# kjenike/panagram

Measured on AMD Instinct MI355X. Metric: anchored k-mers/sec building pan-kmer bitmap, higher is better.
Workload: dtype u64

## Files before the change

panagram_amd/csrc/pg_api.hip:

```cpp
#include "pg_host.h"

thread_local std::string pg::g_err;

int pg::fail(int code, const char *fmt, ...) {
    char buf[512];
    va_list ap;
    va_start(ap, fmt);
    vsnprintf(buf, sizeof buf, fmt, ap);
    va_end(ap);
    g_err = buf;
    return code;
}

extern "C" const char *pg_last_error(void) { return g_err.c_str(); }
int pg_set_error(int code, const char *msg) {
    g_err = msg ? msg : "";
    return code;
}
extern "C" const char *pg_version(void) { return "panagram_hip 0.2 gfx950"; }
extern "C" uint32_t pg_tile_positions(void) { return (uint32_t)PROBE_TILE; }

int pg::use_device(const pg_ctx *c) {
    HIP_TRY(hipSetDevice(c->device));
    return PG_OK;
// ... 699 lines not shown
    }
    return fail(PG_E_CAPACITY, "k-mer counting table keeps overflowing");
    PG_API_END
}

static int insert_keys_dev(pg_table *t, int db_idx, const uint64_t *d_keys, const uint32_t *d_vals, uint64_t n) {
    const int si = 0, w = db_idx;
    if (int r = ensure_room(t, si, n)) return r;
    for (int attempt = 0; attempt < 8; ++attempt) {
        hipStream_t st = t->ctx->stream;
        HIP_TRY(hipMemsetAsync(t->d_counters, 0, 2 * sizeof(unsigned long long), st));
        HIP_TRY(launch_insert_keys(st, t->subs[si].d, w, d_keys, d_vals, n, t->d_counters, MAX_PROBE));
        unsigned long long cnt[2];
        if (int r = read_counters(t, cnt)) return r;
        t->subs[si].count += cnt[0];
        if (cnt[1] == 0) return after_insert(t, si);
        if (int r = grow_after_overflow(t, si, n)) return r;
    }
    return fail(PG_E_CAPACITY, "k-mer table keeps overflowing");
}

extern "C" int pg_table_insert_keys(pg_table *t, int db_idx, const uint64_t *keys, const uint32_t *counters,
                                    uint64_t n) {
    PG_API_BEGIN
    if (!t || (n && (!keys || !counters))) return fail(PG_E_INVALID, "pg_table_insert_keys: NULL argument");
    if (db_idx < 0 || db_idx >= t->ndbs) return fail(PG_E_INVALID, "db index %d out of range (0..%d)", db_idx, t->ndbs - 1);
    if (n == 0) return PG_OK;
    if (int r = use_device(t->ctx)) return r;
    TABLE_WRITER(t);
    DevBuf<uint64_t> dk;
    DevBuf<uint32_t> dv;
    hipError_t e = dk.alloc(n);
    if (e == hipSuccess) e = dv.alloc(n);
    if (e != hipSuccess) return fail(PG_E_HIP, "hipMalloc failed: %s", hipGetErrorString(e));
    int r = PG_OK;
    if (hipMemcpyAsync(dk.get(), keys, n * 8, hipMemcpyHostToDevice, t->ctx->stream) != hipSuccess ||
        hipMemcpyAsync(dv.get(), counters, n * 4, hipMemcpyHostToDevice, t->ctx->stream) != hipSuccess)
        r = fail(PG_E_HIP, "H2D copy of keys failed");
    if (!r) r = insert_keys_dev(t, db_idx, dk.get(), dv.get(), n);
    hipStreamSynchronize(t->ctx->stream);
    return r;
    PG_API_END
}

extern "C" int pg_table_stats(pg_table *t, uint64_t *nkeys, uint64_t *nslots, uint64_t *nbuckets, uint64_t *bytes) {
    PG_API_BEGIN
    if (!t) return fail(PG_E_INVALID, "table is NULL");
    uint64_t a = 0, b = 0, c = 0;
    for (auto &s : t->subs) {
        a += s.count;
        b += s.d.nbuckets * s.d.slots;
        c += s.d.nbuckets;
    }
    if (nkeys) *nkeys = a;
    if (nslots) *nslots = b;
    if (nbuckets) *nbuckets = c;
    if (bytes) {
        uint64_t by = 0;
        for (auto &s2 : t->subs) by += table_bytes(s2.d);
        *bytes = by;
    }
    return PG_OK;
    PG_API_END
}

static int count_spill(pg_table *t, int si, uint64_t *out) {
    hipStream_t st = t->ctx->stream;
    HIP_TRY(hipMemsetAsync(t->d_counters, 0, 2 * sizeof(unsigned long long), st));
    HIP_TRY(launch_count_spill(st, t->subs[si].d, t->d_counters));
    unsigned long long c[2];
    if (int r = read_counters(t, c)) return r;
    *out = c[0];
    return PG_OK;
}

extern "C" int pg_table_rehash(pg_table *t, double keys_per_bucket) {
    PG_API_BEGIN
    if (!t) return fail(PG_E_INVALID, "table is NULL");
    if (!(keys_per_bucket > 0.05 && keys_per_bucket <= 8.0)) return fail(PG_E_INVALID, "keys_per_bucket must be in (0.05, 8]");
    if (int r = use_device(t->ctx)) return r;
    TABLE_WRITER(t);
    if (!t->m_pinned) {
        uint64_t most = 0;
        for (auto &s : t->subs) most = std::max<uint64_t>(most, s.count);
        t->m = minimizer_length((uint32_t)t->k, most, t->max_len, window_cap(t->ngenomes), (uint32_t)t->ngenomes, t->cosched);
    }
    uint32_t slots = 8;
    if (const char *e = getenv("PG_TABLE_SLOTS"))
        if (atoi(e) == 16) slots = 16;
    uint64_t keys = 0, spilled = 0;
    for (size_t si = 0; si < t->subs.size(); ++si) {
        if (t->subs[si].d.layout != LAYOUT_SLOTS) slots = t->subs[si].d.slots;
        const double kpb = std::min(keys_per_bucket * (slots / 8.0), 0.8 * slots);
        if (int r = regrow(t, (int)si, (uint64_t)((double)t->subs[si].count / kpb) + 1, slots)) return r;
        uint64_t sp = 0;
        if (int r = count_spill(t, (int)si, &sp)) return r;
        keys += t->subs[si].count;
        spilled += sp;
    }
    t->spill = keys ? (double)spilled / (double)keys : 0.0;
    return PG_OK;
    PG_API_END
}

extern "C" int pg_table_measure_spill(pg_table *t, double *fraction) {
    PG_API_BEGIN
    if (!t) return fail(PG_E_INVALID, "table is NULL");
    if (int r = use_device(t->ctx)) return r;
    TABLE_WRITER(t);
    uint64_t keys = 0, spilled = 0;
    for (size_t si = 0; si < t->subs.size(); ++si) {
        uint64_t sp = 0;
        if (int r = count_spill(t, (int)si, &sp)) return r;
        keys += t->subs[si].count;
        spilled += sp;
    }
    if (fraction) *fraction = keys ? (double)spilled / (double)keys : 0.0;
    return PG_OK;
    PG_API_END
}

extern "C" int pg_table_spill(const pg_table *t, double *fraction, uint32_t *slots) {
    PG_API_BEGIN
    if (!t) return fail(PG_E_INVALID, "table is NULL");
    if (fraction) *fraction = t->spill;
    if (slots) *slots = t->subs.empty() ? 0 : t->subs[0].d.slots;
    return PG_OK;
    PG_API_END
}

extern "C" int pg_table_export(pg_table *t, int db_idx, uint64_t *keys, uint32_t *counters, uint64_t cap, uint64_t *n) {
    PG_API_BEGIN
    if (!t || !n) return fail(PG_E_INVALID, "pg_table_export: NULL argument");
    if (db_idx < 0 || db_idx >= t->ndbs) return fail(PG_E_INVALID, "db index %d out of range", db_idx);
    if (int r = use_device(t->ctx)) return r;
    const int si = 0, w = db_idx;
    hipStream_t st = t->ctx->stream;
    DevBuf<uint64_t> dk;
    DevBuf<uint32_t> dv;
    if (keys && cap) {
        hipError_t e = dk.alloc(cap);
        if (e == hipSuccess) e = dv.alloc(cap);
        if (e != hipSuccess) return fail(PG_E_HIP, "hipMalloc failed: %s", hipGetErrorString(e));
    }
    int rc = PG_OK;
    unsigned long long cnt[2] = {0, 0};
    if (hipMemsetAsync(t->d_counters, 0, 16, st) != hipSuccess ||
        launch_export(st, t->subs[si].d, w, dk.get(), dv.get(), dk.get() ? cap : 0, t->d_counters) != hipSuccess)
        rc = fail(PG_E_HIP, "export kernel failed");
    if (!rc) rc = read_counters(t, cnt);
    if (!rc && dk.get()) {
        uint64_t m = std::min<uint64_t>(cnt[0], cap);
        if (hipMemcpy(keys, dk.get(), m * 8, hipMemcpyDeviceToHost) != hipSuccess ||
            hipMemcpy(counters, dv.get(), m * 4, hipMemcpyDeviceToHost) != hipSuccess)
            rc = fail(PG_E_HIP, "D2H copy failed");
    }
    *n = cnt[0];
    return rc;
    PG_API_END
}

static TableDesc make_desc(const pg_table *t) {
    TableDesc T;
    memset(&T, 0, sizeof T);
    T.nsub = (uint32_t)t->subs.size();
    for (uint32_t i = 0; i < T.nsub; ++i) T.sub[i] = t->subs[i].d;
    T.ndbs = t->ndbs;
    T.k = t->k;
    T.ngenomes = t->ngenomes;
    return T;
}

struct ResultGeom {
    uint32_t lowres_step = 100;
    uint64_t max_bin_len = 200000;
    uint32_t min_bin_count = 100;
};

static int result_create(pg_ctx *ctx, pg_table *t, int k, uint32_t N, const pg_seqset *sq, uint32_t flags,
                         const ResultGeom &geo, pg_result **out) {
    if (ctx != sq->ctx) return fail(PG_E_INVALID, "table / context and seqset belong to different contexts");
    if (geo.lowres_step < 1 || geo.max_bin_len < 1 || geo.min_bin_count < 1)
        return fail(PG_E_INVALID, "lowres_step, max_bin_len and min_bin_count must be >= 1");
    if (int r = use_device(ctx)) return r;
    const uint32_t nbytes = (N + 7) / 8;
    pg_result *r = new pg_result();
    r->ctx = ctx;
    r->tbl = t;
    r->seqs = sq;
    r->N = N;
    r->k = k;
    if (t) ++t->refs;
    else ++ctx->refs;
    ++const_cast<pg_seqset *>(sq)->refs;
    r->flags = flags;
    r->lowres_step = geo.lowres_step;
    r->d_ad = nullptr;
    r->d_tile_contig = nullptr;
    r->d_out1 = r->d_out100 = nullptr;
    r->d_bins = nullptr;
    r->d_colsums = nullptr;
    r->ev_ok = r->ev_epi = false;
    for (auto &e : r->ev) e = nullptr;
    uint64_t o1 = 0, o100 = 0, bins = 0, tiles = 0;
    std::vector<uint32_t> tile_contig;
    for (uint32_t c = 0; c < sq->n; ++c) {
        const uint64_t len = sq->desc[c].len;
        const uint64_t nk = len >= (uint64_t)k ? len - k + 1 : 0;
        if (nk > 0xFFFFFFF0ull) {
            pg_result_destroy(r);
            return fail(PG_E_INVALID, "contig %u has %llu k-mers; contigs must stay below 2^32 (as in KMC)", c, (unsigned long long)nk);
        }
        AnchorDesc a;
        a.nkmers = (uint32_t)nk;
        uint64_t binlen = geo.max_bin_len;
        if (nk / binlen < geo.min_bin_count) binlen = nk / geo.min_bin_count;
        if (binlen == 0) binlen = 1;
        a.binlen = (uint32_t)binlen;
        a.nbins = (uint32_t)((nk + binlen - 1) / binlen);
        a.out_off = o1;
        a.out100_off = o100;
        a.bin_off = bins;
        a.tile0 = (uint32_t)tiles;
        const uint64_t n100 = (nk + geo.lowres_step - 1) / geo.lowres_step;
        r->nrows100.push_back(n100);
        o1 += (nk * nbytes + 15) & ~15ull;
        o100 += n100 * nbytes;
        bins += a.nbins;
        const uint64_t nt = (nk + PROBE_TILE - 1) / PROBE_TILE;
        for (uint64_t i = 0; i < nt; ++i) tile_contig.push_back(c);
        tiles += nt;
        r->ad.push_back(a);
    }
    if (tiles > 0x7FFFFFFFull) {
        pg_result_destroy(r);
        return fail(PG_E_INVALID, "too many tiles in one launch");
    }
    r->ntiles = (uint32_t)tiles;
    r->out1_bytes = o1;
    r->out100_bytes = o100;
    r->total_bins = bins;
    hipStream_t st = ctx->stream;
    hipError_t e;
    if ((e = hipMalloc(reinterpret_cast<void **>(&r->d_ad), std::max<size_t>(1, r->ad.size()) * sizeof(AnchorDesc))) == hipSuccess &&
        (e = hipMalloc(reinterpret_cast<void **>(&r->d_tile_contig), std::max<size_t>(1, tile_contig.size()) * 4)) == hipSuccess &&
        (e = row_alloc(ctx, (flags & PG_ANCHOR_COLUMNS_ONLY) ? 16 : std::max<uint64_t>(16, o1) + 16, &r->d_out1, &r->out1_cap)) == hipSuccess &&
        (e = hipMalloc(reinterpret_cast<void **>(&r->d_out100), std::max<uint64_t>(16, o100))) == hipSuccess &&
        (e = hipMalloc(reinterpret_cast<void **>(&r->d_bins), std::max<uint64_t>(1, bins) * (N + 1) * 4)) == hipSuccess &&
        (e = hipMalloc(reinterpret_cast<void **>(&r->d_colsums), std::max<size_t>(1, r->ad.size()) * N * 8)) == hipSuccess) {
        if (!r->ad.empty())
            e = hipMemcpyAsync(r->d_ad, r->ad.data(), r->ad.size() * sizeof(AnchorDesc), hipMemcpyHostToDevice, st);
        if (e == hipSuccess && !tile_contig.empty())
            e = hipMemcpyAsync(r->d_tile_contig, tile_contig.data(), tile_contig.size() * 4, hipMemcpyHostToDevice, st);
        if (e == hipSuccess && !t) e = hipMemsetAsync(r->d_out1, 0, std::max<uint64_t>(16, o1), st);
        if (e == hipSuccess) e = hipStreamSynchronize(st);
    }
    if (e != hipSuccess) {
        pg_result_destroy(r);
        return fail(PG_E_HIP, "result allocation failed: %s", hipGetErrorString(e));
    }
    *out = r;
    return PG_OK;
}

extern "C" int pg_result_create(pg_table *t, const pg_seqset *sq, uint32_t flags, pg_result **out) {
    PG_API_BEGIN
    if (!t || !sq || !out) return fail(PG_E_INVALID, "pg_result_create: NULL argument");
    return result_create(t->ctx, t, t->k, (uint32_t)t->ngenomes, sq, flags, ResultGeom(), out);
    PG_API_END
}

extern "C" int pg_result_create_ex(pg_table *t, const pg_seqset *sq, uint32_t flags, uint32_t lowres_step,
                                   uint64_t max_bin_len, uint32_t min_bin_count, pg_result **out) {
    PG_API_BEGIN
    if (!t || !sq || !out) return fail(PG_E_INVALID, "pg_result_create_ex: NULL argument");
    ResultGeom g;
    g.lowres_step = lowres_step;
    g.max_bin_len = max_bin_len;
    g.min_bin_count = min_bin_count;
    return result_create(t->ctx, t, t->k, (uint32_t)t->ngenomes, sq, flags, g, out);
    PG_API_END
}

extern "C" int pg_result_create_rows(pg_ctx *ctx, int k, int ngenomes, const pg_seqset *sq, uint32_t flags,
                                     uint32_t lowres_step, uint64_t max_bin_len, uint32_t min_bin_count, pg_result **out) {
    PG_API_BEGIN
    if (!ctx || !sq || !out) return fail(PG_E_INVALID, "pg_result_create_rows: NULL argument");
    if (k < 1 || k > 32) return fail(PG_E_INVALID, "k=%d unsupported (1..32)", k);
    if (ngenomes < 1) return fail(PG_E_INVALID, "ngenomes must be >= 1");
    ResultGeom g;
    g.lowres_step = lowres_step;
    g.max_bin_len = max_bin_len;
    g.min_bin_count = min_bin_count;
    return result_create(ctx, nullptr, k, (uint32_t)ngenomes, sq, flags | PG_ANCHOR_ROWS_ONLY, g, out);
    PG_API_END
}

extern "C" int pg_result_destroy(pg_result *r) {
    PG_API_BEGIN
    if (!r) return PG_OK;
    hipSetDevice(r->ctx->device);
    hipStreamSynchronize(r->ctx->stream);
    hipStreamSynchronize(r->ctx->aux_stream);
    hipFree(r->d_ad);
    hipFree(r->d_tile_contig);
    row_free(r->ctx, r->d_out1, r->out1_cap);
    hipFree(r->d_out100);
    hipFree(r->d_bins);
    hipFree(r->d_colsums);
    if (r->d_sched) hipFree(r->d_sched);
    if (r->d_ranges) hipFree(r->d_ranges);
    if (r->d_tile_hist) hipFree(r->d_tile_hist);
    if (r->d_tile_cs) hipFree(r->d_tile_cs);
    if (r->d_small) hipFree(r->d_small);
    for (auto e : r->chunk_ev) hipEventDestroy(e);
    for (auto *v : {&r->ev_hist, &r->ev_free})
        for (auto &s : *v)
            for (auto &e : s.e)
                if (e) hipEventDestroy(e);
    pg_table *t = r->tbl;
    pg_ctx *c = r->ctx;
    pg_seqset *sq = const_cast<pg_seqset *>(r->seqs);
    delete r;
    if (t) table_release(t);
    else ctx_release(c);
    seqset_release(sq);
    return PG_OK;
    PG_API_END
}

static int build_chunks(pg_result *r, const uint32_t *sched) {
    r->chunks.clear();
    r->chunks_ready = true;
    if (r->d_ranges) {
        hipFree(r->d_ranges);
        r->d_ranges = nullptr;
    }
    const char *env = getenv("PG_RUN_CHUNKS");
    const uint32_t nbytes = (r->N + 7) / 8;
    uint32_t K = env ? (uint32_t)atoi(env) : ((nbytes == 8 && r->ntiles >= (4u << 20)) ? 16u : 1u);
    const char *mt = getenv("PG_CHUNK_MIN_TILES");
    K = std::min(K, r->ntiles / std::max(1u, mt ? (uint32_t)atoi(mt) : 32768u));
    if (K < 2) return PG_OK;
    std::vector<uint2> ranges;
    for (uint32_t c = 0; c < K; ++c) {
        pg_result::Chunk ch;
        ch.s0 = (uint32_t)((uint64_t)r->ntiles * c / K);
        ch.s1 = (uint32_t)((uint64_t)r->ntiles * (c + 1) / K);
        ch.r0 = (uint32_t)ranges.size();
        ch.tiles = ch.s1 - ch.s0;
        if (!sched) {
            ranges.push_back(make_uint2(ch.s0, ch.s1));
        } else {
            std::vector<uint2> runs;
            for (uint32_t i = ch.s0; i < ch.s1; ++i) {
                if (!runs.empty() && runs.back().y == sched[i]) ++runs.back().y;
                else runs.push_back(make_uint2(sched[i], sched[i] + 1));
            }
            std::sort(runs.begin(), runs.end(), [](const uint2 &a, const uint2 &b) { return a.x < b.x; });
            for (const uint2 &u : runs) {
                if (ranges.size() > ch.r0 && ranges.back().y == u.x) ranges.back().y = u.y;
                else ranges.push_back(u);
            }
        }
        ch.nr = (uint32_t)ranges.size() - ch.r0;
        if (ch.nr > 512) {
            r->chunks.clear();
            return PG_OK;
        }
        r->chunks.push_back(ch);
    }
    HIP_TRY(hipMalloc(reinterpret_cast<void **>(&r->d_ranges), ranges.size() * sizeof(uint2)));
    HIP_TRY(hipMemcpy(r->d_ranges, ranges.data(), ranges.size() * sizeof(uint2), hipMemcpyHostToDevice));
    while (r->chunk_ev.size() < r->chunks.size()) {
        hipEvent_t e;
        HIP_TRY(hipEventCreateWithFlags(&e, hipEventDisableTiming));
        r->chunk_ev.push_back(e);
    }
    return PG_OK;
}

static int coschedule(pg_result *r, const uint32_t *contig_group, uint32_t piece_tiles, const uint32_t *range_first,
                      uint32_t nranges, const uint32_t *contig_class = nullptr) {
    if (int e = use_device(r->ctx)) return e;
    hipStream_t st = r->ctx->stream;
    HIP_TRY(hipStreamSynchronize(st));
    HIP_TRY(hipStreamSynchronize(r->ctx->aux_stream));
    if (r->d_sched) {
        hipFree(r->d_sched);
        r->d_sched = nullptr;
    }
    r->sched_bounds.clear();
    r->chunks.clear();
    r->chunks_ready = false;
    if (!contig_group || r->ntiles == 0) return PG_OK;
    const bool auto_piece = piece_tiles == 0;
    const size_t nc = r->ad.size();
    std::vector<uint32_t> firsts;
    if (range_first && nranges) {
        for (uint32_t i = 0; i < nranges; ++i) {
            if (range_first[i] >= nc || (i && range_first[i] <= range_first[i - 1]) || (!i && range_first[0] != 0))
                return fail(PG_E_INVALID, "pg_result_coschedule_ranges: range starts must begin at contig 0 and increase");
            firsts.push_back(range_first[i]);
        }
    } else {
        firsts.push_back(0);
    }
    firsts.push_back((uint32_t)nc);
    struct Piece {
        double at;
        uint32_t g, first;
    };
    std::vector<uint32_t> sched;
    sched.reserve(r->ntiles);
    std::vector<std::vector<uint32_t>> members;
    if (contig_class) {
        std::vector<std::pair<uint32_t, uint32_t>> byclass;
        for (size_t c = 0; c < nc; ++c) byclass.emplace_back(contig_class[c], (uint32_t)c);
        std::stable_sort(byclass.begin(), byclass.end(), [](auto &x, auto &y) { return x.first < y.first; });
        for (size_t i = 0; i < byclass.size(); ++i) {
            if (i == 0 || byclass[i].first != byclass[i - 1].first) members.emplace_back();
            members.back().push_back(byclass[i].second);
        }
        r->sched_bounds.push_back(0);
    } else {
        for (size_t ri = 0; ri + 1 < firsts.size(); ++ri) {
            members.emplace_back();
            for (uint32_t c = firsts[ri]; c < firsts[ri + 1]; ++c) members.back().push_back(c);
            r->sched_bounds.push_back(r->ad[firsts[ri]].tile0);
        }
    }
    for (const auto &mem : members) {
        uint32_t ngroups = 0;
        for (uint32_t c : mem) ngroups = std::max(ngroups, contig_group[c] + 1);
        std::vector<std::vector<uint32_t>> tiles(ngroups);
        for (uint32_t c : mem) {
            const uint32_t nt = (uint32_t)(((uint64_t)r->ad[c].nkmers + PROBE_TILE - 1) / PROBE_TILE);
            for (uint32_t i = 0; i < nt; ++i) tiles[contig_group[c]].push_back(r->ad[c].tile0 + i);
        }
        if (auto_piece) piece_tiles = ngroups <= 32 ? 64u : std::max(8u, 512u / ngroups);
        std::vector<Piece> pieces;
        for (uint32_t g = 0; g < ngroups; ++g) {
            const size_t np = (tiles[g].size() + piece_tiles - 1) / piece_tiles;
            for (size_t i = 0; i < np; ++i) pieces.push_back({(double)i / (double)np, g, (uint32_t)(i * piece_tiles)});
        }
        std::stable_sort(pieces.begin(), pieces.end(), [](const Piece &x, const Piece &y) { return x.at < y.at; });
        for (const Piece &p : pieces) {
            const size_t end = std::min<size_t>(tiles[p.g].size(), (size_t)p.first + piece_tiles);
            for (size_t i = p.first; i < end; ++i) sched.push_back(tiles[p.g][i]);
        }
    }
    r->sched_bounds.push_back(r->ntiles);
    if (sched.size() != r->ntiles) return fail(PG_E_INVALID, "internal: schedule does not cover the tiles");
    HIP_TRY(hipMalloc(reinterpret_cast<void **>(&r->d_sched), (size_t)r->ntiles * 4));
    HIP_TRY(hipMemcpyAsync(r->d_sched, sched.data(), (size_t)r->ntiles * 4, hipMemcpyHostToDevice, st));
    HIP_TRY(hipStreamSynchronize(st));
    if (!(r->flags & PG_ANCHOR_ROWS_ONLY)) return build_chunks(r, sched.data());
    return PG_OK;
}

extern "C" int pg_result_coschedule(pg_result *r, const uint32_t *contig_group, uint32_t piece_tiles) {
    PG_API_BEGIN
    if (!r) return fail(PG_E_INVALID, "result is NULL");
    return coschedule(r, contig_group, piece_tiles, nullptr, 0);
    PG_API_END
}

extern "C" int pg_result_coschedule_classes(pg_result *r, const uint32_t *contig_group, const uint32_t *contig_class,
                                            uint32_t piece_tiles) {
    PG_API_BEGIN
    if (!r) return fail(PG_E_INVALID, "result is NULL");
    if (contig_group && !contig_class) return fail(PG_E_INVALID, "pg_result_coschedule_classes: contig_class is NULL");
    return coschedule(r, contig_group, piece_tiles, nullptr, 0, contig_class);
    PG_API_END
}

extern "C" int pg_result_coschedule_ranges(pg_result *r, const uint32_t *contig_group, uint32_t piece_tiles,
                                           const uint32_t *range_first_contig, uint32_t nranges) {
    PG_API_BEGIN
    if (!r) return fail(PG_E_INVALID, "result is NULL");
    return coschedule(r, contig_group, piece_tiles, range_first_contig, nranges);
    PG_API_END
}

static int enqueue_epilogue(pg_result *r, hipStream_t st) {
    const uint32_t N = r->N;
    HIP_TRY(hipMemsetAsync(r->d_bins, 0, std::max<uint64_t>(1, r->total_bins) * (N + 1) * 4, st));
    HIP_TRY(hipMemsetAsync(r->d_colsums, 0, std::max<size_t>(1, r->ad.size()) * N * 8, st));
    const uint32_t kflags = (r->flags & PG_ANCHOR_COLSUMS) | (r->lowres_step == 100 ? 0u : 2u);
    HIP_TRY(launch_rows_epilogue(st, N, r->d_ad, r->d_tile_contig, r->ntiles, r->d_out1, r->d_out100, r->d_bins,
                                 r->d_colsums, kflags));
    if (r->lowres_step != 100)
        HIP_TRY(launch_lowres(st, N, r->d_ad, r->d_tile_contig, r->ntiles, r->d_out1, r->d_out100, r->lowres_step));
    return PG_OK;
}

static bool fuse_enabled() {
    const char *e = getenv("PG_FUSE_STATS");
    return e && *e == '1';
}
static bool fuse_table_ok(const TableDesc &T, uint32_t N) {
    return T.nsub == 1 && T.ngenomes == N && !(T.sub[0].layout == LAYOUT_SLOTS && T.sub[0].slots != 8);
}
static int prepare_fuse(pg_result *r, const TableDesc &T) {
    if (r->fuse_state) return PG_OK;
    r->fuse_state = -1;
    const uint32_t nbytes = (r->N + 7) / 8;
    if (!fuse_rows_ok(nbytes) || !fuse_table_ok(T, r->N)) return PG_OK;
    std::vector<uint2> small;
    uint64_t small_tiles = 0, fused_tiles = 0;
    for (const AnchorDesc &a : r->ad) {
        const uint32_t nt = (uint32_t)(((uint64_t)a.nkmers + PROBE_TILE - 1) / PROBE_TILE);
        if (!nt) continue;
        if (a.binlen >= (uint32_t)PROBE_TILE) {
            fused_tiles += nt;
            continue;
        }
        small_tiles += nt;
        if (!small.empty() && small.back().y == a.tile0) small.back().y = a.tile0 + nt;
        else small.push_back(make_uint2(a.tile0, a.tile0 + nt));
    }
    if (!fused_tiles || small.size() > 16384) return PG_OK;
    const size_t hb = (size_t)r->ntiles * fuse_hist_words(r->N) * 4, cb = (size_t)r->ntiles * fuse_cs_words(r->N) * 4;
    if (hipMalloc(reinterpret_cast<void **>(&r->d_tile_hist), hb) != hipSuccess || hipMalloc(reinterpret_cast<void **>(&r->d_tile_cs), cb) != hipSuccess ||
        (!small.empty() && hipMalloc(reinterpret_cast<void **>(&r->d_small), small.size() * sizeof(uint2)) != hipSuccess)) {
        (void)hipGetLastError();
        if (r->d_tile_hist) hipFree(r->d_tile_hist);
        if (r->d_tile_cs) hipFree(r->d_tile_cs);
        r->d_tile_hist = r->d_tile_cs = nullptr;
        return PG_OK;
    }
    if (!small.empty()) HIP_TRY(hipMemcpy(r->d_small, small.data(), small.size() * sizeof(uint2), hipMemcpyHostToDevice));
    r->n_small = (uint32_t)small.size();
    r->small_tiles = (uint32_t)small_tiles;
    r->fuse_state = 1;
    return PG_OK;
}
static FuseArgs fuse_args(const pg_result *r) {
    FuseArgs fa;
    fa.out100 = r->lowres_step == 100 ? r->d_out100 : nullptr;
    fa.tile_hist = r->d_tile_hist;
    fa.tile_cs = r->d_tile_cs;
    fa.ngenomes = r->N;
    fa.hw = fuse_hist_words(r->N);
    fa.csw = fuse_cs_words(r->N);
    return fa;
}
static int enqueue_fused_epilogue(pg_result *r, hipStream_t st, const FuseArgs &fa) {
    const uint32_t N = r->N;
    HIP_TRY(hipMemsetAsync(r->d_bins, 0, std::max<uint64_t>(1, r->total_bins) * (N + 1) * 4, st));
    HIP_TRY(hipMemsetAsync(r->d_colsums, 0, std::max<size_t>(1, r->ad.size()) * N * 8, st));
    HIP_TRY(launch_tile_reduce(st, fa, r->d_ad, r->d_tile_contig, r->ntiles, r->d_bins, r->d_colsums, (r->flags & PG_ANCHOR_COLSUMS) ? 1u : 0u));
    const uint32_t kflags = (r->flags & PG_ANCHOR_COLSUMS) | (r->lowres_step == 100 ? 0u : 2u);
    if (r->n_small)
        HIP_TRY(launch_rows_epilogue(st, N, r->d_ad, r->d_tile_contig, r->ntiles, r->d_out1, r->d_out100, r->d_bins, r->d_colsums, kflags,
                                     r->d_small, r->n_small, r->small_tiles));
    if (r->lowres_step != 100)
        HIP_TRY(launch_lowres(st, N, r->d_ad, r->d_tile_contig, r->ntiles, r->d_out1, r->d_out100, r->lowres_step));
    return PG_OK;
}

int pg::join_result(pg_result *r) {
    if (r->ev_epi) HIP_TRY(hipStreamWaitEvent(r->ctx->stream, r->ev[3], 0));
    return PG_OK;
}

static int fold_timing(pg_result *r, const pg_result::EvSet &s) {
    HIP_TRY(hipEventSynchronize(s.e[s.epi ? 3 : 1]));
    float a = 0, b = 0;
    if (s.probe) {
        HIP_TRY(hipEventElapsedTime(&a, s.e[0], s.e[1]));
        r->probe_ms_sum += a;
        ++r->probe_runs;
    }
    if (s.epi) {
        HIP_TRY(hipEventElapsedTime(&b, s.e[2], s.e[3]));
        r->epi_ms_sum += b;
        ++r->epi_runs;
    }
    return PG_OK;
}

int pg::next_events(pg_result *r, bool probe) {
    if (r->ev_hist.size() >= EV_RING) {
        if (r->hist_skip) --r->hist_skip;
        else if (int e = fold_timing(r, r->ev_hist.front())) return e;
        r->ev_free.push_back(r->ev_hist.front());
        r->ev_hist.erase(r->ev_hist.begin());
    }
    pg_result::EvSet s;
    if (!r->ev_free.empty()) {
        s = r->ev_free.back();
        r->ev_free.pop_back();
    } else {
        for (auto &e : s.e) {
            e = nullptr;
            HIP_TRY(hipEventCreate(&e));
        }
    }
    s.probe = probe;
    s.epi = false;
    r->ev_hist.push_back(s);
    for (int i = 0; i < 4; ++i) r->ev[i] = s.e[i];
    return PG_OK;
}

static int contig_tiles(const pg_result *r, uint32_t first, uint32_t n, uint32_t *t0, uint32_t *nt) {
    if ((uint64_t)first + n > r->ad.size()) return fail(PG_E_INVALID, "contigs %u..%u out of range (the result has %zu)", first, first + n, r->ad.size());
    if (n == 0) {
        *t0 = *nt = 0;
        return PG_OK;
    }
    const AnchorDesc &a = r->ad[first], &z = r->ad[first + n - 1];
    *t0 = a.tile0;
    *nt = z.tile0 + (uint32_t)(((uint64_t)z.nkmers + PROBE_TILE - 1) / PROBE_TILE) - a.tile0;
    return PG_OK;
}

static bool sched_covers(const pg_result *r, uint32_t t0, uint32_t nt) {
    if (!r->d_sched) return false;
    const auto &b = r->sched_bounds;
    return std::binary_search(b.begin(), b.end(), t0) && std::binary_search(b.begin(), b.end(), t0 + nt);
}

static int run_chunks(pg_result *r, const TableDesc &T) {
    hipStream_t st = r->ctx->stream, aux = r->ctx->aux_stream;
    if (const char *e = getenv("PG_CHUNK_SAME_STREAM"); e && *e == '1') aux = st;
    const uint32_t N = r->N;
    const uint32_t kflags = (r->flags & PG_ANCHOR_COLSUMS) | (r->lowres_step == 100 ? 0u : 2u);
    HIP_TRY(hipEventRecord(r->ev[0], st));
    for (size_t c = 0; c < r->chunks.size(); ++c) {
        const pg_result::Chunk &ch = r->chunks[c];
        HIP_TRY(launch_anchor(st, T, r->seqs->d_seqw, r->seqs->d_nmw, r->seqs->d_has_n, r->seqs->d_desc, r->d_ad, r->d_tile_contig,
                              r->d_sched, ch.s0, ch.s1 - ch.s0, r->d_out1, r->out1_bytes, 0));
        HIP_TRY(hipEventRecord(r->chunk_ev[c], st));
        HIP_TRY(hipStreamWaitEvent(aux, r->chunk_ev[c], 0));
        if (c == 0) {
            HIP_TRY(hipEventRecord(r->ev[2], aux));
            HIP_TRY(hipMemsetAsync(r->d_bins, 0, std::max<uint64_t>(1, r->total_bins) * (N + 1) * 4, aux));
            HIP_TRY(hipMemsetAsync(r->d_colsums, 0, std::max<size_t>(1, r->ad.size()) * N * 8, aux));
        }
        HIP_TRY(launch_rows_epilogue(aux, N, r->d_ad, r->d_tile_contig, r->ntiles, r->d_out1, r->d_out100, r->d_bins, r->d_colsums,
                                     kflags, r->d_ranges + ch.r0, ch.nr, ch.tiles));
    }
    HIP_TRY(hipEventRecord(r->ev[1], st));
    if (r->lowres_step != 100)
        HIP_TRY(launch_lowres(aux, N, r->d_ad, r->d_tile_contig, r->ntiles, r->d_out1, r->d_out100, r->lowres_step));
    HIP_TRY(hipEventRecord(r->ev[3], aux));
    r->ev_ok = r->ev_epi = true;
    r->ev_hist.back().epi = true;
    return PG_OK;
}

static int anchor_run(pg_result *r, uint32_t tile_base, uint32_t ntiles, bool whole, uint32_t columns_width = 0,
                      void *d_columns = nullptr) {
    pg_table *t = r->tbl;
    if (!t) return fail(PG_E_INVALID, "this result is a rows container (pg_result_create_rows): it has no table to probe");
    if (int e = use_device(r->ctx)) return e;
    hipStream_t st = r->ctx->stream, aux = r->ctx->aux_stream;
    if (int e = join_result(r)) return e;
    if (int e = next_events(r, true)) return e;
    TableDesc T = make_desc(t);
    const bool stats = whole && !columns_width && !(r->flags & PG_ANCHOR_ROWS_ONLY);
    bool fuse = false;
    if (stats && fuse_enabled()) {
        if (int e = prepare_fuse(r, T)) return e;
        fuse = r->fuse_state == 1 && fuse_table_ok(T, r->N);
    }
    if (stats && !fuse) {
        if (!r->chunks_ready)
            if (int e = build_chunks(r, nullptr)) return e;
        if (r->chunks.size() > 1) return run_chunks(r, T);
    }
    const FuseArgs fa = fuse_args(r);
    HIP_TRY(hipEventRecord(r->ev[0], st));
    HIP_TRY(launch_anchor(st, T, r->seqs->d_seqw, r->seqs->d_nmw, r->seqs->d_has_n, r->seqs->d_desc, r->d_ad,
                          r->d_tile_contig, sched_covers(r, tile_base, ntiles) ? r->d_sched : nullptr, tile_base, ntiles,
                          columns_width ? static_cast<uint8_t *>(d_columns) : r->d_out1, r->out1_bytes, columns_width, fuse ? &fa : nullptr));
    HIP_TRY(hipEventRecord(r->ev[1], st));
    r->ev_ok = true;
    r->ev_epi = false;
    if (stats) {
        HIP_TRY(hipStreamWaitEvent(aux, r->ev[1], 0));
        HIP_TRY(hipEventRecord(r->ev[2], aux));
        if (fuse) {
            if (int e = enqueue_fused_epilogue(r, aux, fa)) return e;
            ++r->fused_runs;
        } else if (int e = enqueue_epilogue(r, aux)) return e;
        HIP_TRY(hipEventRecord(r->ev[3], aux));
        r->ev_epi = true;
        r->ev_hist.back().epi = true;
    }
    return PG_OK;
}

extern "C" int pg_anchor_run(pg_result *r) {
    PG_API_BEGIN
    if (!r) return fail(PG_E_INVALID, "result is NULL");
    if (r->flags & PG_ANCHOR_COLUMNS_ONLY) return fail(PG_E_INVALID, "a PG_ANCHOR_COLUMNS_ONLY result has no rows: use pg_anchor_run_columns_range");
    return anchor_run(r, 0, r->ntiles, true);
    PG_API_END
}

extern "C" int pg_anchor_run_range(pg_result *r, uint32_t first_contig, uint32_t ncontigs) {
    PG_API_BEGIN
    if (!r) return fail(PG_E_INVALID, "result is NULL");
    if (r->flags & PG_ANCHOR_COLUMNS_ONLY) return fail(PG_E_INVALID, "a PG_ANCHOR_COLUMNS_ONLY result has no rows: use pg_anchor_run_columns_range");
    if (!(r->flags & PG_ANCHOR_ROWS_ONLY)) return fail(PG_E_INVALID, "pg_anchor_run_range needs a PG_ANCHOR_ROWS_ONLY result");
    uint32_t t0, nt;
    if (int e = contig_tiles(r, first_contig, ncontigs, &t0, &nt)) return e;
    return anchor_run(r, t0, nt, false);
    PG_API_END
}

extern "C" int pg_result_columns_direct(const pg_result *r, uint32_t width) {
    PG_API_BEGIN
    if (!r || !r->tbl) return 0;
    const pg_table *t = r->tbl;
    return t->subs.size() == 1 && t->subs[0].d.layout == LAYOUT_SLOTS && t->subs[0].d.W == 1 && t->subs[0].d.slots == 8 &&
           t->ngenomes <= 8 && width <= 8 && (int)width >= t->ngenomes;
    PG_API_END
}

extern "C" int pg_anchor_run_columns_range(pg_result *r, uint32_t first_contig, uint32_t ncontigs, uint32_t width, void *d_dst) {
    PG_API_BEGIN
    if (!r || !d_dst) return fail(PG_E_INVALID, "pg_anchor_run_columns_range: NULL argument");
    if (!pg_result_columns_direct(r, width))
        return fail(PG_E_INVALID, "pg_anchor_run_columns_range: needs a table of up to 8 genomes (8-slot lines) and width in ngenomes..8");
    uint32_t t0, nt;
    if (int e = contig_tiles(r, first_contig, ncontigs, &t0, &nt)) return e;
    return anchor_run(r, t0, nt, false, width, d_dst);
    PG_API_END
}

extern "C" int pg_result_timing(pg_result *r, float *probe_ms, float *epilogue_ms) {
    PG_API_BEGIN
    if (!r) return fail(PG_E_INVALID, "result is NULL");
    if (!r->ev_ok) return fail(PG_E_INVALID, "pg_anchor_run has not been called on this result");
    if (int e = use_device(r->ctx)) return e;
    HIP_TRY(hipEventSynchronize(r->ev[r->ev_epi ? 3 : 1]));
    float a = 0, b = 0;
    HIP_TRY(hipEventElapsedTime(&a, r->ev[0], r->ev[1]));
    if (r->ev_epi) HIP_TRY(hipEventElapsedTime(&b, r->ev[2], r->ev[3]));
    if (probe_ms) *probe_ms = a;
    if (epilogue_ms) *epilogue_ms = b;
    return PG_OK;
    PG_API_END
}

extern "C" int pg_result_fused_runs(const pg_result *r, uint32_t *n) {
    PG_API_BEGIN
    if (!r || !n) return fail(PG_E_INVALID, "pg_result_fused_runs: NULL argument");
    *n = r->fused_runs;
    return PG_OK;
    PG_API_END
}

extern "C" int pg_result_timing_reset(pg_result *r) {
    PG_API_BEGIN
    if (!r) return fail(PG_E_INVALID, "result is NULL");
    while (r->ev_hist.size() > 1) {
        r->ev_free.push_back(r->ev_hist.front());
        r->ev_hist.erase(r->ev_hist.begin());
    }
    r->hist_skip = r->ev_hist.size();
    r->probe_ms_sum = r->epi_ms_sum = 0;
    r->probe_runs = r->epi_runs = 0;
    return PG_OK;
    PG_API_END
}

extern "C" int pg_result_timing_mean(pg_result *r, double *probe_ms, double *epilogue_ms, uint32_t *nruns) {
    PG_API_BEGIN
    if (!r) return fail(PG_E_INVALID, "result is NULL");
    if (int e = use_device(r->ctx)) return e;
    const double a0 = r->probe_ms_sum, b0 = r->epi_ms_sum;
    const uint32_t pn0 = r->probe_runs, en0 = r->epi_runs;
    int rc = PG_OK;
    for (size_t i = r->hist_skip; i < r->ev_hist.size() && !rc; ++i) rc = fold_timing(r, r->ev_hist[i]);
    if (!rc) {
        if (probe_ms) *probe_ms = r->probe_runs ? r->probe_ms_sum / r->probe_runs : 0.0;
        if (epilogue_ms) *epilogue_ms = r->epi_runs ? r->epi_ms_sum / r->epi_runs : 0.0;
        if (nruns) *nruns = r->probe_runs;
    }
    r->probe_ms_sum = a0;
    r->epi_ms_sum = b0;
    r->probe_runs = pn0;
    r->epi_runs = en0;
    return rc;
    PG_API_END
}

extern "C" uint64_t pg_result_columns_bytes(const pg_result *r, uint32_t width) {
    return r ? (uint64_t)r->ntiles * (PROBE_TILE / 8) * width : 0;
}

extern "C" uint64_t pg_result_columns_bytes_range(const pg_result *r, uint32_t width, uint32_t first_contig, uint32_t ncontigs) {
    uint32_t t0, nt;
    if (!r || contig_tiles(r, first_contig, ncontigs, &t0, &nt)) return 0;
    return (uint64_t)nt * (PROBE_TILE / 8) * width;
}

extern "C" int pg_result_extract_columns_range(pg_result *r, uint32_t g0, uint32_t width, uint32_t first_contig,
                                               uint32_t ncontigs, void *d_dst) {
    PG_API_BEGIN
    if (!r || !d_dst) return fail(PG_E_INVALID, "pg_result_extract_columns: NULL argument");
    if (!r->ev_ok && !r->rows_valid) return fail(PG_E_INVALID, "the result holds no rows yet");
    uint32_t t0, nt;
    if (int e = contig_tiles(r, first_contig, ncontigs, &t0, &nt)) return e;
    if (int e = use_device(r->ctx)) return e;
    HIP_TRY(launch_cols_extract(r->ctx->stream, r->N, r->d_ad, r->d_tile_contig, t0, nt, r->d_out1, g0, width, d_dst));
    return PG_OK;
    PG_API_END
}

extern "C" int pg_result_extract_columns(pg_result *r, uint32_t g0, uint32_t width, void *d_dst) {
    PG_API_BEGIN
    if (!r) return fail(PG_E_INVALID, "pg_result_extract_columns: NULL argument");
    return pg_result_extract_columns_range(r, g0, width, 0, (uint32_t)r->ad.size(), d_dst);
    PG_API_END
}

extern "C" int pg_result_merge_columns_range(pg_result *r, const void *d_src, uint32_t part0, uint32_t nparts, uint32_t per,
                                             uint32_t first_contig, uint32_t ncontigs, int accumulate,
                                             uint64_t part_stride_bytes) {
    PG_API_BEGIN
    if (!r || !d_src) return fail(PG_E_INVALID, "pg_result_merge_columns: NULL argument");
    if (per == 0 || nparts == 0) return fail(PG_E_INVALID, "pg_result_merge_columns: empty partition");
    uint32_t t0, nt;
    if (int e = contig_tiles(r, first_contig, ncontigs, &t0, &nt)) return e;
    const uint64_t own = (uint64_t)nt * (PROBE_TILE / 8) * per;
    if (part_stride_bytes == 0) part_stride_bytes = own;
    if (part_stride_bytes < own || part_stride_bytes % 8) return fail(PG_E_INVALID, "pg_result_merge_columns_range: bad block stride");
    if (int e = use_device(r->ctx)) return e;
    if (int e = join_result(r)) return e;
    HIP_TRY(launch_cols_merge(r->ctx->stream, r->N, r->d_ad, r->d_tile_contig, t0, nt, r->d_out1, d_src, part0, nparts,
                              part_stride_bytes / 8, per, accumulate ? 1u : 0u));
    r->rows_valid = true;
    return PG_OK;
    PG_API_END
}

extern "C" int pg_result_merge_columns(pg_result *r, const void *d_src, uint32_t nparts, uint32_t per) {
    PG_API_BEGIN
    if (!r) return fail(PG_E_INVALID, "pg_result_merge_columns: NULL argument");
    return pg_result_merge_columns_range(r, d_src, 0, nparts, per, 0, (uint32_t)r->ad.size(), 0, 0);
    PG_API_END
}

extern "C" int pg_rows_epilogue(pg_result *r) {
    PG_API_BEGIN
    if (!r) return fail(PG_E_INVALID, "result is NULL");
    if (int e = use_device(r->ctx)) return e;
    if (int e = join_result(r)) return e;
    hipStream_t st = r->ctx->stream;
    if (int e = next_events(r, false)) return e;
    HIP_TRY(hipEventRecord(r->ev[0], st));
    HIP_TRY(hipEventRecord(r->ev[1], st));
    HIP_TRY(hipEventRecord(r->ev[2], st));
    if (int e = enqueue_epilogue(r, st)) return e;
    HIP_TRY(hipEventRecord(r->ev[3], st));
    r->ev_ok = true;
    r->ev_epi = true;
    r->ev_hist.back().epi = true;
    return PG_OK;
    PG_API_END
}

extern "C" int pg_result_contig_info(const pg_result *r, uint32_t idx, uint64_t *nkmers, uint64_t *nrows100,
                                     uint32_t *nbins, uint32_t *binlen) {
    PG_API_BEGIN
    if (!r) return fail(PG_E_INVALID, "result is NULL");
    if (idx >= r->ad.size()) return fail(PG_E_INVALID, "contig %u out of range", idx);
    if (nkmers) *nkmers = r->ad[idx].nkmers;
    if (nrows100) *nrows100 = r->nrows100[idx];
    if (nbins) *nbins = r->ad[idx].nbins;
    if (binlen) *binlen = r->ad[idx].binlen;
    return PG_OK;
    PG_API_END
}

extern "C" int pg_result_contigs_small(pg_result *r, uint32_t first, uint32_t ncontigs, uint64_t *nkmers, uint64_t *nrows100,
                                       uint32_t *nbins, uint32_t *binlen, uint32_t *bins, uint64_t bins_words) {
    PG_API_BEGIN
    if (!r) return fail(PG_E_INVALID, "result is NULL");
    if ((uint64_t)first + ncontigs > r->ad.size()) return fail(PG_E_INVALID, "contigs %u..%u out of range", first, first + ncontigs);
    uint64_t rows = 0;
    for (uint32_t i = 0; i < ncontigs; ++i) {
        const AnchorDesc &a = r->ad[first + i];
        if (nkmers) nkmers[i] = a.nkmers;
        if (nrows100) nrows100[i] = r->nrows100[first + i];
        if (nbins) nbins[i] = a.nbins;
        if (binlen) binlen[i] = a.binlen;
        rows += a.nbins;
    }
    if (!bins || ncontigs == 0) return PG_OK;
    const uint64_t N1 = (uint64_t)r->N + 1;
    if (bins_words != rows * N1) return fail(PG_E_INVALID, "pg_result_contigs_small: %llu words for %llu bin rows of %llu", (unsigned long long)bins_words, (unsigned long long)rows, (unsigned long long)N1);
    if (rows == 0) return PG_OK;
    if (int e = use_device(r->ctx)) return e;
    if (int e = join_result(r)) return e;
    hipStream_t st = r->ctx->stream;
    HIP_TRY(hipMemcpyAsync(bins, r->d_bins + r->ad[first].bin_off * N1, rows * N1 * 4, hipMemcpyDeviceToHost, st));
    HIP_TRY(hipStreamSynchronize(st));
    return PG_OK;
    PG_API_END
}

extern "C" int pg_result_download(pg_result *r, uint32_t idx, uint8_t *bitmap1, uint8_t *bitmap100, uint32_t *bins) {
    PG_API_BEGIN
    if (!r) return fail(PG_E_INVALID, "result is NULL");
    if (idx >= r->ad.size()) return fail(PG_E_INVALID, "contig %u out of range", idx);
    if (int e = use_device(r->ctx)) return e;
    if (int e = join_result(r)) return e;
    hipStream_t st = r->ctx->stream;
    const AnchorDesc &a = r->ad[idx];
    const uint32_t N = r->N, nbytes = (N + 7) / 8;
    if (bitmap1 && a.nkmers)
        HIP_TRY(hipMemcpyAsync(bitmap1, r->d_out1 + a.out_off, (uint64_t)a.nkmers * nbytes, hipMemcpyDeviceToHost, st));
    if (bitmap100 && r->nrows100[idx])
        HIP_TRY(hipMemcpyAsync(bitmap100, r->d_out100 + a.out100_off, r->nrows100[idx] * nbytes, hipMemcpyDeviceToHost, st));
    if (bins && a.nbins)
        HIP_TRY(hipMemcpyAsync(bins, r->d_bins + a.bin_off * (N + 1), (uint64_t)a.nbins * (N + 1) * 4, hipMemcpyDeviceToHost, st));
    HIP_TRY(hipStreamSynchronize(st));
    return PG_OK;
    PG_API_END
}

extern "C" int pg_result_colsums(pg_result *r, uint64_t *colsums) {
    PG_API_BEGIN
    if (!r || !colsums) return fail(PG_E_INVALID, "pg_result_colsums: NULL argument");
    if (!(r->flags & PG_ANCHOR_COLSUMS)) return fail(PG_E_INVALID, "result was created without PG_ANCHOR_COLSUMS");
    if (int e = use_device(r->ctx)) return e;
    if (int e = join_result(r)) return e;
    hipStream_t st = r->ctx->stream;
    const size_t N = r->N, nc = r->ad.size();
    std::vector<uint64_t> all(std::max<size_t>(1, nc) * N, 0);
    if (nc) {
        HIP_TRY(hipMemcpyAsync(all.data(), r->d_colsums, nc * N * 8, hipMemcpyDeviceToHost, st));
        HIP_TRY(hipStreamSynchronize(st));
    }
    for (size_t g = 0; g < N; ++g) colsums[g] = 0;
    for (size_t c = 0; c < nc; ++c)
        for (size_t g = 0; g < N; ++g) colsums[g] += all[c * N + g];
    return PG_OK;
    PG_API_END
}

extern "C" int pg_result_contig_colsums(pg_result *r, uint32_t idx, uint32_t ncontigs, uint64_t *colsums) {
    PG_API_BEGIN
    if (!r || !colsums) return fail(PG_E_INVALID, "pg_result_contig_colsums: NULL argument");
    if (!(r->flags & PG_ANCHOR_COLSUMS)) return fail(PG_E_INVALID, "result was created without PG_ANCHOR_COLSUMS");
    if ((uint64_t)idx + ncontigs > r->ad.size()) return fail(PG_E_INVALID, "contigs %u..%u out of range", idx, idx + ncontigs);
    if (ncontigs == 0) return PG_OK;
    if (int e = use_device(r->ctx)) return e;
    if (int e = join_result(r)) return e;
    hipStream_t st = r->ctx->stream;
    const size_t N = r->N;
    HIP_TRY(hipMemcpyAsync(colsums, r->d_colsums + (size_t)idx * N, (size_t)ncontigs * N * 8, hipMemcpyDeviceToHost, st));
    HIP_TRY(hipStreamSynchronize(st));
    return PG_OK;
    PG_API_END
}

extern "C" int pg_result_device_ptrs(pg_result *r, void **d1, uint64_t *b1, void **d100, uint64_t *b100) {
    PG_API_BEGIN
    if (!r) return fail(PG_E_INVALID, "result is NULL");
    if (d1) *d1 = r->d_out1;
    if (b1) *b1 = r->out1_bytes;
    if (d100) *d100 = r->d_out100;
    if (b100) *b100 = r->out100_bytes;
    return PG_OK;
    PG_API_END
}

extern "C" int pg_anchor_contig(pg_table *t, const char *ascii, uint64_t len, uint8_t *bitmap1, uint8_t *bitmap100,
                                uint32_t *bins, uint64_t *colsums, uint64_t *nkmers) {
    PG_API_BEGIN
    if (!t || (len && !ascii)) return fail(PG_E_INVALID, "pg_anchor_contig: NULL argument");
    if (nkmers) *nkmers = len >= (uint64_t)t->k ? len - t->k + 1 : 0;
    if (colsums) memset(colsums, 0, (size_t)t->ngenomes * 8);
    if (len < (uint64_t)t->k) return PG_OK;
    pg_seqset *sq = nullptr;
    pg_result *res = nullptr;
    int rc = pg_seqset_create(t->ctx, 1, &len, &sq);
    if (!rc) rc = pg_seqset_load_host(sq, 0, ascii, len);
    if (!rc) rc = pg_result_create(t, sq, colsums ? PG_ANCHOR_COLSUMS : 0, &res);
    if (!rc) rc = pg_anchor_run(res);
    if (!rc) rc = pg_result_download(res, 0, bitmap1, bitmap100, bins);
    if (!rc && colsums) rc = pg_result_colsums(res, colsums);
    pg_result_destroy(res);
    pg_seqset_destroy(sq);
    return rc;
// ... 28 lines not shown
```

panagram_amd/csrc/pg_host.h:

```cpp
#pragma once
#include "../../include/panagram_hip.h"
#include "pg_kernels.h"
#include "pg_guard.h"

#include <algorithm>
#include <atomic>
#include <condition_variable>
#include <cmath>
#include <cstdarg>
#include <cstdio>
#include <cstdlib>
#include <cstring>
#include <memory>
#include <mutex>
#include <string>
#include <system_error>
#include <thread>
#include <vector>

using namespace pg;

#define PG_INTERNAL __attribute__((visibility("hidden")))

#define HIP_TRY(expr)                                                                          \
    do {                                                                                       \
        hipError_t e_ = (expr);                                                                \
        if (e_ != hipSuccess)                                                                  \
            return fail(PG_E_HIP, "%s failed: %s (%s:%d)", #expr, hipGetErrorString(e_), __FILE__, __LINE__); \
    } while (0)

struct pg_ctx {
    int device;
    hipStream_t own_stream;
    hipStream_t stream;
    hipStream_t aux_stream;
    std::atomic<int> refs{0};
    bool dead = false;
    struct DfSet {
        uint8_t *d_slots[2] = {nullptr, nullptr}, *d_packed[2] = {nullptr, nullptr}, *h_slots[2] = {nullptr, nullptr};
        uint32_t *d_sizes[2] = {nullptr, nullptr}, *d_offs[2] = {nullptr, nullptr}, *h_sizes[2] = {nullptr, nullptr};
        uint32_t *d_crc = nullptr, *d_hist = nullptr;
        void *d_code = nullptr;
        bool ready = false, busy = false;
    } df[4];
    std::mutex df_mu;
    std::condition_variable df_cv;
    struct RowBuf {
        uint8_t *p;
        uint64_t cap;
    };
    std::vector<RowBuf> row_cache;
    std::mutex row_mu;
};

struct SubHost {
    SubTable d;
    uint64_t count;
};

struct pg_table {
    pg_ctx *ctx;
    int k, ngenomes, ndbs;
    uint32_t m;
    bool m_pinned = false;
    uint32_t cosched = 0;
    uint64_t expected = 0;
    double load0 = 0.375;
    uint64_t first_len = 0;
    uint64_t max_len = 0;
    std::vector<SubHost> subs;
    unsigned long long *d_counters;
    unsigned long long *h_counters = nullptr;
    uint32_t *d_tile0 = nullptr;
    size_t tile0_cap = 0;
    double spill = 0;
    std::atomic<int> refs{0};
    bool dead = false;
    std::mutex write_mu;
};
#define TABLE_WRITER(t) std::lock_guard<std::mutex> writer_guard_((t)->write_mu)

struct pg_seqset {
    pg_ctx *ctx;
    uint32_t n;
    std::vector<SeqDesc> desc;
    uint64_t total_words;
    uint64_t *d_seqw;
    uint32_t *d_nmw;
    uint32_t *d_has_n;
    SeqDesc *d_desc;
    void *d_stage;
    size_t stage_cap;
    std::vector<std::string> names;
    std::atomic<int> refs{0};
    bool dead = false;
};

struct pg_result {
    pg_ctx *ctx;
    pg_table *tbl;
    const pg_seqset *seqs;
    uint32_t N;
    int k;
    uint32_t flags;
    uint32_t lowres_step = 100;
    std::vector<AnchorDesc> ad;
    std::vector<uint64_t> nrows100;
    AnchorDesc *d_ad;
    uint32_t *d_tile_contig;
    uint32_t *d_sched = nullptr;
    std::vector<uint32_t> sched_bounds;
    uint32_t ntiles;
    uint8_t *d_out1;
    uint64_t out1_bytes;
    uint64_t out1_cap = 0;
    uint8_t *d_out100;
    uint64_t out100_bytes;
    uint32_t *d_bins;
    uint64_t total_bins;
    unsigned long long *d_colsums;
    hipEvent_t ev[4];
    bool ev_ok, ev_epi;
    bool rows_valid = false;
    struct EvSet {
        hipEvent_t e[4];
        bool probe, epi;
    };
    std::vector<EvSet> ev_hist, ev_free;
    struct Chunk {
        uint32_t s0, s1, r0, nr, tiles;
    };
    std::vector<Chunk> chunks;
    uint2 *d_ranges = nullptr;
    bool chunks_ready = false;
    std::vector<hipEvent_t> chunk_ev;
    size_t hist_skip = 0;
    double probe_ms_sum = 0, epi_ms_sum = 0;
    uint32_t probe_runs = 0, epi_runs = 0;
    int fuse_state = 0;
    uint32_t *d_tile_hist = nullptr, *d_tile_cs = nullptr;
    uint2 *d_small = nullptr;
    uint32_t n_small = 0, small_tiles = 0;
    uint32_t fused_runs = 0;
};
static constexpr size_t EV_RING = 128;

template <class T>
struct DevBuf {
    T *p = nullptr;
    DevBuf() = default;
    DevBuf(DevBuf &&o) noexcept : p(o.p) { o.p = nullptr; }
    ~DevBuf() {
        if (p) hipFree(p);
    }
    hipError_t alloc(size_t count) { return hipMalloc(reinterpret_cast<void **>(&p), count * sizeof(T)); }
    hipError_t upload(const std::vector<T> &h, hipStream_t st) {
        const hipError_t e = alloc(h.size());
        return e != hipSuccess ? e : hipMemcpyAsync(p, h.data(), h.size() * sizeof(T), hipMemcpyHostToDevice, st);
    }
    T *get() const { return p; }
};
template <class T>
struct PinBuf {
    T *p = nullptr;
    PinBuf() = default;
    PinBuf(PinBuf &&o) noexcept : p(o.p) { o.p = nullptr; }
    ~PinBuf() {
        if (p) hipHostFree(p);
    }
    hipError_t alloc(size_t count, unsigned flags) { return hipHostMalloc(reinterpret_cast<void **>(&p), count * sizeof(T), flags); }
    T *get() const { return p; }
};
struct Stream {
    hipStream_t s = nullptr;
    Stream() = default;
    Stream(Stream &&o) noexcept : s(o.s) { o.s = nullptr; }
    ~Stream() {
        if (!s) return;
        hipStreamSynchronize(s);
        hipStreamDestroy(s);
    }
    hipError_t create() { return hipStreamCreateWithFlags(&s, hipStreamNonBlocking); }
    hipStream_t get() const { return s; }
};
struct Event {
    hipEvent_t ev = nullptr;
    Event() = default;
    Event(Event &&o) noexcept : ev(o.ev) { o.ev = nullptr; }
    ~Event() {
        if (ev) hipEventDestroy(ev);
    }
    hipError_t create(unsigned flags) { return hipEventCreateWithFlags(&ev, flags); }
    hipEvent_t get() const { return ev; }
};

static constexpr uint32_t MAX_PROBE = 512;
static constexpr double GROW_AT = 0.55;
#ifndef PG_INLINE_LAYOUT
#define PG_INLINE_LAYOUT 1
#endif
static constexpr double TARGET_LOAD = 0.375;
static constexpr double HARD_LOAD = 0.85;

struct Windows {
    uint32_t n = 0;
    uint64_t longest = 0;
    std::vector<uint64_t> se;
    DevBuf<uint64_t> d_se;
    hipError_t upload(hipStream_t st) { return d_se.upload(se, st); }
    const uint64_t *base() const { return d_se.get(); }
    const uint64_t *starts() const { return d_se.get() + n; }
    const uint64_t *ends() const { return d_se.get() + 2 * (size_t)n; }
};

namespace pg {
extern PG_INTERNAL thread_local std::string g_err;
PG_INTERNAL int fail(int code, const char *fmt, ...);
PG_INTERNAL int use_device(const pg_ctx *c);
PG_INTERNAL int check_step(const pg_result *r, int step);
PG_INTERNAL void ctx_release(pg_ctx *c);
PG_INTERNAL hipError_t row_alloc(pg_ctx *c, uint64_t bytes, uint8_t **out, uint64_t *cap);
PG_INTERNAL void row_free(pg_ctx *c, uint8_t *p, uint64_t cap);
PG_INTERNAL uint32_t window_cap(int ngenomes = 0);
PG_INTERNAL int read_counters(pg_table *t, unsigned long long out[2]);
PG_INTERNAL int ensure_room(pg_table *t, int si, uint64_t incoming);
PG_INTERNAL int grow_after_overflow(pg_table *t, int si, uint64_t incoming);
PG_INTERNAL int after_insert(pg_table *t, int si);
PG_INTERNAL int join_result(pg_result *r);
PG_INTERNAL int next_events(pg_result *r, bool probe);
PG_INTERNAL void seqset_release(pg_seqset *s);
PG_INTERNAL int check_window_call(const pg_result *r, int step, uint32_t stride, uint32_t n, const char *fn, const char *nouns);
PG_INTERNAL int gather_windows(const pg_result *r, int step, uint32_t stride, uint32_t n, const uint32_t *contig, const uint64_t *starts,
                               const uint64_t *ends, const char *noun, Windows &w);
PG_INTERNAL uint32_t valid_word(uint32_t N, uint32_t d);
PG_INTERNAL std::vector<uint32_t> mask_words(uint32_t N, const uint32_t *words, uint32_t if_null);
PG_INTERNAL uint32_t pieces_for(uint64_t longest, uint32_t nwin, uint32_t cap);
PG_INTERNAL int cut_chunks(const char *fn, uint32_t nwin, const uint64_t *starts, const uint64_t *ends, uint32_t chunk_rows,
                           std::vector<uint2> &chunks, std::vector<uint64_t> *first = nullptr);
PG_INTERNAL void df_free_buffers(pg_ctx::DfSet &d);
}
```

Baseline: 229.4 billion.

## Zero epilogue buffers on aux stream early and run repeat epilogues inline

The memsets that zero bins and colsums now start on the aux stream as soon as the run begins (after ev[0]) instead of after the probe, so they overlap with the probe kernel. When the same result is run again back-to-back on a context and the fused path is not used, the epilogue is enqueued directly on the main stream after the probe. This avoids the cross-stream event hop, and join_result skips the extra wait. The change adds a fifth event and a last_run tracker on the context, plus more complex event bookkeeping in the timing ring.

Result: no change. 229.7 billion, median of 4 (+0.1%).

```diff
diff --git a/panagram_amd/csrc/pg_api.hip b/panagram_amd/csrc/pg_api.hip
--- a/panagram_amd/csrc/pg_api.hip
+++ b/panagram_amd/csrc/pg_api.hip
@@ -1025,6 +1025,8 @@
     hipSetDevice(r->ctx->device);
     hipStreamSynchronize(r->ctx->stream);
     hipStreamSynchronize(r->ctx->aux_stream);
+    pg_result *self = r;
+    r->ctx->last_run.compare_exchange_strong(self, nullptr);
     hipFree(r->d_ad);
     hipFree(r->d_tile_contig);
     row_free(r->ctx, r->d_out1, r->out1_cap);
@@ -1206,10 +1208,16 @@
     PG_API_END
 }
 
-static int enqueue_epilogue(pg_result *r, hipStream_t st) {
+static int enqueue_zero(pg_result *r, hipStream_t st) {
+    HIP_TRY(hipMemsetAsync(r->d_bins, 0, std::max<uint64_t>(1, r->total_bins) * (r->N + 1) * 4, st));
+    HIP_TRY(hipMemsetAsync(r->d_colsums, 0, std::max<size_t>(1, r->ad.size()) * r->N * 8, st));
+    return PG_OK;
+}
+
+static int enqueue_epilogue(pg_result *r, hipStream_t st, hipEvent_t zeroed = nullptr) {
     const uint32_t N = r->N;
-    HIP_TRY(hipMemsetAsync(r->d_bins, 0, std::max<uint64_t>(1, r->total_bins) * (N + 1) * 4, st));
-    HIP_TRY(hipMemsetAsync(r->d_colsums, 0, std::max<size_t>(1, r->ad.size()) * N * 8, st));
+    if (zeroed) HIP_TRY(hipStreamWaitEvent(st, zeroed, 0));
+    else if (int e = enqueue_zero(r, st)) return e;
     const uint32_t kflags = (r->flags & PG_ANCHOR_COLSUMS) | (r->lowres_step == 100 ? 0u : 2u);
     HIP_TRY(launch_rows_epilogue(st, N, r->d_ad, r->d_tile_contig, r->ntiles, r->d_out1, r->d_out100, r->d_bins,
                                  r->d_colsums, kflags));
@@ -1269,10 +1277,9 @@
     fa.csw = fuse_cs_words(r->N);
     return fa;
 }
-static int enqueue_fused_epilogue(pg_result *r, hipStream_t st, const FuseArgs &fa) {
+static int enqueue_fused_epilogue(pg_result *r, hipStream_t st, const FuseArgs &fa, hipEvent_t zeroed) {
     const uint32_t N = r->N;
-    HIP_TRY(hipMemsetAsync(r->d_bins, 0, std::max<uint64_t>(1, r->total_bins) * (N + 1) * 4, st));
-    HIP_TRY(hipMemsetAsync(r->d_colsums, 0, std::max<size_t>(1, r->ad.size()) * N * 8, st));
+    HIP_TRY(hipStreamWaitEvent(st, zeroed, 0));
     HIP_TRY(launch_tile_reduce(st, fa, r->d_ad, r->d_tile_contig, r->ntiles, r->d_bins, r->d_colsums, (r->flags & PG_ANCHOR_COLSUMS) ? 1u : 0u));
     const uint32_t kflags = (r->flags & PG_ANCHOR_COLSUMS) | (r->lowres_step == 100 ? 0u : 2u);
     if (r->n_small)
@@ -1284,7 +1291,7 @@
 }
 
 int pg::join_result(pg_result *r) {
-    if (r->ev_epi) HIP_TRY(hipStreamWaitEvent(r->ctx->stream, r->ev[3], 0));
+    if (r->ev_epi && !(r->epi_inline && r->epi_stream == r->ctx->stream)) HIP_TRY(hipStreamWaitEvent(r->ctx->stream, r->ev[3], 0));
     return PG_OK;
 }
 
@@ -1297,7 +1304,7 @@
         ++r->probe_runs;
     }
     if (s.epi) {
-        HIP_TRY(hipEventElapsedTime(&b, s.e[2], s.e[3]));
+        HIP_TRY(hipEventElapsedTime(&b, s.e[s.e2], s.e[3]));
         r->epi_ms_sum += b;
         ++r->epi_runs;
     }
@@ -1323,8 +1330,10 @@
     }
     s.probe = probe;
     s.epi = false;
+    s.e2 = 2;
     r->ev_hist.push_back(s);
-    for (int i = 0; i < 4; ++i) r->ev[i] = s.e[i];
+    for (int i = 0; i < 5; ++i) r->ev[i] = s.e[i];
+    r->epi_inline = false;
     return PG_OK;
 }
 
@@ -1383,6 +1392,7 @@
     hipStream_t st = r->ctx->stream, aux = r->ctx->aux_stream;
     if (int e = join_result(r)) return e;
     if (int e = next_events(r, true)) return e;
+    const bool repeat = r->ctx->last_run.exchange(r) == r;
     TableDesc T = make_desc(t);
     const bool stats = whole && !columns_width && !(r->flags & PG_ANCHOR_ROWS_ONLY);
     bool fuse = false;
@@ -1404,14 +1414,26 @@
     r->ev_ok = true;
     r->ev_epi = false;
     if (stats) {
-        HIP_TRY(hipStreamWaitEvent(aux, r->ev[1], 0));
-        HIP_TRY(hipEventRecord(r->ev[2], aux));
+        HIP_TRY(hipStreamWaitEvent(aux, r->ev[0], 0));
+        if (int e = enqueue_zero(r, aux)) return e;
+        HIP_TRY(hipEventRecord(r->ev[4], aux));
+        const bool inl = repeat && !fuse;
+        hipStream_t ps = inl ? st : aux;
+        if (inl) {
+            r->ev[2] = r->ev[1];
+            r->ev_hist.back().e2 = 1;
+        } else {
+            HIP_TRY(hipStreamWaitEvent(aux, r->ev[1], 0));
+            HIP_TRY(hipEventRecord(r->ev[2], aux));
+        }
         if (fuse) {
-            if (int e = enqueue_fused_epilogue(r, aux, fa)) return e;
+            if (int e = enqueue_fused_epilogue(r, ps, fa, r->ev[4])) return e;
             ++r->fused_runs;
-        } else if (int e = enqueue_epilogue(r, aux)) return e;
-        HIP_TRY(hipEventRecord(r->ev[3], aux));
+        } else if (int e = enqueue_epilogue(r, ps, r->ev[4])) return e;
+        HIP_TRY(hipEventRecord(r->ev[3], ps));
         r->ev_epi = true;
+        r->epi_inline = inl;
+        r->epi_stream = st;
         r->ev_hist.back().epi = true;
     }
     return PG_OK;
diff --git a/panagram_amd/csrc/pg_host.h b/panagram_amd/csrc/pg_host.h
--- a/panagram_amd/csrc/pg_host.h
+++ b/panagram_amd/csrc/pg_host.h
@@ -29,11 +29,13 @@
             return fail(PG_E_HIP, "%s failed: %s (%s:%d)", #expr, hipGetErrorString(e_), __FILE__, __LINE__); \
     } while (0)
 
+struct pg_result;
 struct pg_ctx {
     int device;
     hipStream_t own_stream;
     hipStream_t stream;
     hipStream_t aux_stream;
+    std::atomic<pg_result *> last_run{nullptr};
     std::atomic<int> refs{0};
     bool dead = false;
     struct DfSet {
@@ -119,12 +121,15 @@
     uint32_t *d_bins;
     uint64_t total_bins;
     unsigned long long *d_colsums;
-    hipEvent_t ev[4];
+    hipEvent_t ev[5];
     bool ev_ok, ev_epi;
+    bool epi_inline = false;
+    hipStream_t epi_stream = nullptr;
     bool rows_valid = false;
     struct EvSet {
-        hipEvent_t e[4];
+        hipEvent_t e[5];
         bool probe, epi;
+        int e2;
     };
     std::vector<EvSet> ev_hist, ev_free;
     struct Chunk {
```
